# mackelab/poisson-gpfa

Hardware: AMD Instinct MI355X
Metric: EM iterations/sec (higher is better)
Workload: dtype f64

## Files before the change

poisson-gpfa_amd/csrc/core.hip:

```cpp
#include "ctx.h"
#include "model.h"
#include "dual.h"

using namespace pgpfa;

thread_local std::string g_err;
thread_local unsigned long long g_fail_count = 0;

int fail(const char* fmt, ...) {
  char buf[1024];
  va_list ap;
  va_start(ap, fmt);
  vsnprintf(buf, sizeof(buf), fmt, ap);
  va_end(ap);
  g_err = buf;
  ++g_fail_count;
  return 1;
}

int ensure_hbuf(pgpfa_ctx* c, size_t len) {
  if (len <= c->hbuf_len) return 0;
  if (c->hbuf) hipHostFree(c->hbuf);
  c->hbuf = nullptr;
  HIPC(hipHostMalloc((void**)&c->hbuf, len * sizeof(double)));
// ... 842 lines not shown
  c->info["arena_bytes"] = 0.0;
  c->info["last_eps_wt_norm"] = 0.0;
  c->info["last_eps_wt_rms"] = 0.0;
  c->info["last_split_cov"] = 0.0;
  c->info["last_syrk_tile"] = 0.0;
  c->info["last_split_sps"] = 0.0;
  c->info["last_cross_kernel"] = 0.0;
  c->info["last_mix_form"] = 0.0;
  c->info["last_yt_mix_fused"] = 0.0;
  c->info["last_cov_f32"] = 0.0;
  c->info["last_cov_f32_fallbacks"] = 0.0;
  for (const char* k : {"plan_ms_total", "plans", "set_params_calls", "last_retry_ms", "last_dense_retries", "last_param_step", "last_param_step_prev",
                        "last_fallback_no_descent", "last_fallback_line_search", "last_fallback_outer_cap", "arena_grow_ms_total", "last_cold_restarts"}) c->info[k] = 0.0;
  *out = c;
  return 0;
}

int pgpfa_destroy(pgpfa_ctx* c) {
  if (!c) return 0;
  hipSetDevice(c->device);
  if (c->st) hipStreamSynchronize(c->st);
  if (c->comm) ncclCommDestroy(c->comm);
  for (void* p : c->allocs) hipFree(p);
  if (c->vsmgp) hipFree(c->vsmgp);
  if (c->Flr32) hipFree(c->Flr32);
  if (c->lam_keep) hipFree(c->lam_keep);
  if (c->split_buf) hipFree(c->split_buf);
  if (c->Yhi) hipFree(c->Yhi);
  if (c->trial_len) hipFree(c->trial_len);
  if (c->obs) hipFree(c->obs);
  if (c->trunc_q) hipFree(c->trunc_q);
  arena_release(c);
  if (c->hbuf) hipHostFree(c->hbuf);
  if (c->dl_stage) hipHostFree(c->dl_stage);
  if (c->hibuf) hipHostFree(c->hibuf);
  if (c->ring) hipHostFree(c->ring);
  if (c->h_pcg) hipHostFree(c->h_pcg);
  if (c->h_seq) hipHostFree(c->h_seq);
  for (auto e : c->prof.pool) hipEventDestroy(e);
  if (c->st2) { hipStreamSynchronize(c->st2); hipStreamDestroy(c->st2); }
  if (c->tau_pin) hipHostFree(c->tau_pin);
  if (c->ev_tau_fork) hipEventDestroy(c->ev_tau_fork);
  if (c->ev_tau_done) hipEventDestroy(c->ev_tau_done);
  if (c->ev_fork) hipEventDestroy(c->ev_fork);
  if (c->ev_join) hipEventDestroy(c->ev_join);
  if (c->st) hipStreamDestroy(c->st);
  delete c;
  return 0;
}

int pgpfa_set_option(pgpfa_ctx* c, const char* key, double v) {
  if (!c || !key) return fail("null argument");
  const std::string k(key);
  if (k == "newton_xtol") c->xtol = v;
  else if (k == "newton_max_iter") c->max_iter = (int)v;
  else if (k == "use_mfma") {
    const bool was = c->mfma;
    c->mfma = (v != 0.0);
    if (c->have_params && c->rank_gran != 16 && was != c->mfma)
      CHK(pgpfa_set_params(c, std::vector<double>(c->hC).data(), std::vector<double>(c->hd).data(), std::vector<double>(c->htau).data()));
  }
  else if (k == "cd_mfma") c->cd_mfma = (v != 0.0);
  else if (k == "cd_hess_mfma") c->cd_hess_mfma = (v != 0.0);
  else if (k == "cross_kernel") c->cross_kernel = (v != 0.0);
  else if (k == "cd_debug") c->cd_debug = (int)v;
  else if (k == "pcg_fused") c->pcg_fused = (int)v;
  else if (k == "pcg_w32") c->pcg_w32 = (v != 0.0);
  else if (k == "pcg_form") c->pcg_form = (int)v;
  else if (k == "pcg_vec32") c->pcg_vec32 = (int)v;
  else if (k == "pcg_rx32") c->pcg_rx32 = (int)v;
  else if (k == "pcg_adapt") c->pcg_adapt = (int)v;
  else if (k == "pcg_xcd") c->pcg_xcd = (int)v;
  else if (k == "mt_fill") c->mt_fill = (int)v;
  else if (k == "overlap_factors") c->overlap_factors = (int)v;
  else if (k == "mix_slot") c->mix_slot = (int)v;
  else if (k == "yt_mix") c->yt_mix = (v != 0.0);
  else if (k == "pivchol_pairs") c->pivchol_pairs = (v != 0.0);
  else if (k == "vsm_b4") c->vsm_b4 = (int)v;
  else if (k == "poisson_tiles") c->poisson_tiles = (int)v;
  else if (k == "yt_mix_dbg") c->yt_mix_dbg = (int)v;
  else if (k == "yt_mix_dma") c->yt_mix_dma = (v != 0.0);
  else if (k == "syrk_dbg") c->syrk_dbg = (int)v;
  else if (k == "syrk_tile") c->syrk_tile = (int)v;
  else if (k == "mix_wide") c->mix_wide = (int)v;
  else if (k == "thin_products") {
    const bool was = c->thin_products >= 2;
    c->thin_products = (int)v;
    if (c->have_params && c->rank_gran != 16 && was != (c->thin_products >= 2))
      CHK(pgpfa_set_params(c, std::vector<double>(c->hC).data(), std::vector<double>(c->hd).data(), std::vector<double>(c->htau).data()));
  }
  else if (k == "copy_kernels") c->copy_kernels = (v != 0.0);
  else if (k == "chord") c->chord = (v != 0.0);
  else if (k == "shared_pcg") c->shared_pcg = (v != 0.0);
  else if (k == "time_newton") c->time_newton = (v != 0.0);
  else if (k == "pcg_trace") c->pcg_trace = (v != 0.0);
  else if (k == "measure_mix") { c->measure_mix = (v != 0.0); c->info["last_eps_wt_norm"] = 0.0; c->info["last_eps_wt_rms"] = 0.0; }
  else if (k == "pcg_retire") c->pcg_retire = (v != 0.0);
  else if (k == "split_cov") c->split_cov = (v != 0.0);
  else if (k == "split_max_norm") c->split_max_norm = v;
  else if (k == "cov_mode") c->cov_mode = (int)v;
  else if (k == "lowrank_tol") {
    const bool changed = c->lr_tol != v;
    c->lr_tol = v;
    if (c->have_params && changed)
      CHK(pgpfa_set_params(c, std::vector<double>(c->hC).data(), std::vector<double>(c->hd).data(), std::vector<double>(c->htau).data()));
  }
  else if (k == "keep_trial_vsmgp") c->keep_trial_vsmgp = (v != 0.0);
  else if (k == "dual_lowrank") c->dual_lowrank = (v != 0.0);
  else if (k == "dual_f32") c->dual_f32 = (int)v;
  else if (k == "laplace_f32") { if (v != 0.0 && v != 1.0 && v != 2.0) return fail("laplace_f32 is 0, 1 or 2"); c->laplace_f32 = (int)v; }
  else if (k == "dual_masked") { if (v != 0.0 && v != 1.0) return fail("dual_masked is 0 or 1"); c->dual_masked = (int)v; }
  else if (k == "laplace_evidence") { if (v != 0.0 && v != 1.0) return fail("laplace_evidence is 0 or 1"); c->laplace_evidence = (int)v; }
  else if (k == "sample_chunk_trials") { if (v < 0.0 || v != std::floor(v)) return fail("sample_chunk_trials is a count of trials, or 0"); c->sample_chunk = (int)v; }
  else if (k == "rates_chunk_trials") { if (v < 0.0 || v != std::floor(v)) return fail("rates_chunk_trials is a count of trials, or 0"); c->rates_chunk = (int)v; }
  else if (k == "slab_row_align") c->slab_row_align = (v != 0.0);
  else if (k == "vsm_mfma") c->vsm_mfma = (v != 0.0);
  else if (k == "dual_gemm") c->dual_gemm = (v != 0.0);
  else if (k == "extrapolate_start") c->extrapolate = (v != 0.0);
  else if (k == "extrapolate_beta") c->extrapolate_beta = v;
  else if (k == "extrapolate_guard") c->extrapolate_guard = v;
  else if (k == "start_guard") c->start_guard = (v != 0.0);
  else if (k == "shared_min") c->shared_min = (int)v;
  else if (k == "pcg_inner") c->pcg_inner_max = std::max(1, (int)v);
  else if (k == "pcg_eta0") c->pcg_eta0 = v;
  else if (k == "splitk_target") c->splitk_target = std::max(1, (int)v);
  else if (k == "small_tile_below") c->small_tile_below = (int)v;
  else if (k == "f32_tile64") c->f32_tile64 = (int)v;
  else if (k == "splitk_below64") c->splitk_below64 = (int)v;
  else if (k == "pcg_outer_max") c->pcg_outer_max = (int)v;
  else if (k == "chord_xtol") c->chord_xtol = v;
  else if (k == "chord_rho") c->chord_rho = v;
  else if (k == "chord_max_step") c->chord_max_step = v;
  else if (k == "chord_max") c->chord_max = (int)v;
  else if (k == "chunk_trials") { if (c->B > 0) return fail("chunk_trials must be set before the first E-step"); c->chunk_opt = (int)v; }
  else if (k == "workspace_headroom") c->arena_headroom = std::max(1.0, v);
  else if (k == "rank_gran") { if (v != 4.0 && v != 8.0 && v != 16.0) return fail("rank_gran is 4, 8 or 16"); c->rank_gran = (int)v; if (c->have_params) CHK(pgpfa_set_params(c, std::vector<double>(c->hC).data(), std::vector<double>(c->hd).data(), std::vector<double>(c->htau).data())); }
  else if (k == "workspace_pool") { if (c->arena_cap > 0) return fail("workspace_pool must be set before the first E-step"); c->use_pool = (v != 0.0); }
  else if (k == "workspace_grow_budget_ms") c->grow_budget_ms = v;
  else if (k == "workspace_grow_floor_slots") c->grow_floor_slots = std::max(1, (int)v);
  else if (k == "workspace_granule_mb") c->vmm_granule = (size_t)std::max(2.0, v) << 20;
  else if (k == "workspace_vmm") { if (c->arena_cap > 0) return fail("workspace_vmm must be set before the first E-step"); c->vmm = (v != 0.0) ? 0 : -1; }
  else if (k == "eps_noise") {
    const bool changed = c->eps != v;
    c->eps = v;
    if (c->have_params && changed)
      CHK(pgpfa_set_params(c, std::vector<double>(c->hC).data(), std::vector<double>(c->hd).data(), std::vector<double>(c->htau).data()));
  }
  else if (k == "profile") {
    if (v != 0.0) {
      prof_collect(c);
      c->prof.ms.clear(); c->prof.flops.clear(); c->prof.count.clear(); c->prof.max_ms.clear(); c->prof.max_flops.clear(); c->prof.shapes.clear();
      HIPC(hipSetDevice(c->device));
      const size_t want = 2 * (256 + 64) + 2;
      while (c->prof.pool.size() < want) {
        hipEvent_t e;
        HIPC(hipEventCreate(&e));
        c->prof.pool.push_back(e);
        c->prof.idle.push_back(e);
      }
      for (int rep = 0; rep < 8; ++rep)
        for (hipEvent_t e : c->prof.idle) HIPC(hipEventRecord(e, c->st));
      HIPC(hipStreamSynchronize(c->st));
    }
    c->prof.on = (v != 0.0);
    c->prof.configured = c->prof.on;
    c->prof.only_tag = (v == 2.0) ? TAG_GEMM : (v == 3.0) ? TAG_MIX : -1;
// ... 452 lines not shown
```

poisson-gpfa_amd/csrc/cov.hip:

```cpp
#include "ctx.h"
#include "model.h"
#include "split.h"
#include "ytmix.h"

using namespace pgpfa;

template <typename TIN>
void launch_post_vsm(pgpfa_ctx* c, const TIN* Mt, long long sM, int ncol, int ns, int full_range, const int* roff = nullptr, int ts = 0) {
  const int T = c->T, p = c->p;
  if (ts <= 0) ts = T;
  if (p > 10 && c->vsm_mfma) {
    const int CB = post_vsm_mfma_cb(p, sizeof(TIN) == 4);
    if (p <= 20 && c->vsm_b4) {
      constexpr int VW = 16 / (int)sizeof(TIN);
      const bool vec = c->vsm_b4 >= 2 && T % VW == 0 && ts % VW == 0 && c->ld % VW == 0 && sM % VW == 0 && (((size_t)Mt) & 15) == 0;
      auto go = [&](auto nbk, auto vv) {
        constexpr int NBK = decltype(nbk)::value;
        constexpr bool VEC = decltype(vv)::value;
        const size_t lds4 = (size_t)CB * post_vsm_b4_cs(p, VEC) * sizeof(TIN);
        constexpr int BINS = VEC ? 64 : 32;
        (void)hipFuncSetAttribute(reinterpret_cast<const void*>(&post_vsm_b4_kernel<NBK, TIN, VEC>), hipFuncAttributeMaxDynamicSharedMemorySize, (int)lds4);
        hipLaunchKernelGGL((post_vsm_b4_kernel<NBK, TIN, VEC>), dim3((T + BINS - 1) / BINS, ns), dim3(512), lds4, c->st, Mt, sM, c->ld, ncol, T, p, c->vsm,
                           c->ident, c->trial_of_slot, full_range, CB, roff, (int)GBN, ts);
      };
// ... 35 lines not shown
  }
}


int ensure_mt_clean(pgpfa_ctx* c) {
  if (!c->mt_dirty) return 0;
  HIPC(hipMemsetAsync(c->ws.Mt, 0, (size_t)c->ws.sM * c->B * sizeof(double), c->st));
  c->mt_dirty = false;
  return 0;
}

int ensure_vsmgp_buffer(pgpfa_ctx* c) {
  if (c->vsmgp) return 0;
  const size_t bytes = (size_t)c->R * c->p * c->T * c->T * sizeof(double);
  void* ptr = nullptr;
  hipError_t e = hipMalloc(&ptr, bytes);
  if (e != hipSuccess) { (void)hipGetLastError(); return fail("hipMalloc(%zu bytes) for the per-trial post_vsmGP blocks failed: %s", bytes, hipGetErrorString(e)); }
  e = hipMemsetAsync(ptr, 0, bytes, c->st);
  if (e != hipSuccess) { hipFree(ptr); return fail("hipMemset failed: %s", hipGetErrorString(e)); }
  c->vsmgp = reinterpret_cast<double*>(ptr);
  c->bytes += bytes;
  return 0;
}

int ensure_evidence_buffers(pgpfa_ctx* c) {
  if (!c->ldet_buf) CHK(dmalloc(c, &c->ldet_buf, (size_t)c->B * c->T + 16));
  if (!c->evid_ld) CHK(dmalloc(c, &c->evid_ld, (size_t)c->B));
  return 0;
}

static int posterior_blocks_dense(pgpfa_ctx* c, int nb, double diag_scale, bool want_vsmgp, double* ld_dev) {
  const int T = c->T, p = c->p;
  c->info["last_cov_f32"] = 0.0;
  CHK(ensure_mt_clean(c));
  c->last_cov_lowrank = false;
  CHK(assemble(c, c->ident, nb, diag_scale));
  CHK(factor(c, c->ws, c->ident, nb));
  if (ld_dev) {
    double ldk = 0.0;
    for (double v : c->logdetK) ldk += v;
    hipLaunchKernelGGL(evidence_logdet_kernel, dim3(nb), dim3(256), 0, c->st, (const double*)nullptr, 0, c->ws.H, (long long)c->ws.sH, c->ld, c->npad, ldk, ld_dev);
  }
  CHK(inverse_t(c, c->ws, c->ident, nb));
  if (want_vsmgp) {
    CHK(ensure_vsmgp_buffer(c));
    for (int k = 0; k < p; ++k) {
      const int kal = (k * T) / 16 * 16;
      GemmP g{};
      g.A = c->ws.Mt + (size_t)kal * c->ld + (size_t)k * T; g.sA = c->ws.sM; g.lda = c->ld;
      g.B = g.A; g.sB = c->ws.sM; g.ldb = c->ld;
      g.C = c->ws.H; g.sC = c->ws.sH; g.ldc = T;
      g.M = T; g.N = T; g.K = c->npad - kal; g.alpha = 1.0; g.beta = 0.0;
      g.slots = c->ident; g.nbatch = nb; g.mode = GEMM_LOWER; g.kflags = KF_BEGIN_MAXRC;
      CHK(gemm(c, false, g));
      hipLaunchKernelGGL(scatter_vsmgp_kernel, dim3((unsigned)(((size_t)T * T + 255) / 256), nb), dim3(256), 0, c->st, c->ws.H, c->ws.sH, c->vsmgp,
                         T, p, k, c->trial_of_slot);
    }
  }
  prof_begin(c, TAG_VSM, (double)nb * c->npad * c->npad * p);
  launch_post_vsm(c, (const double*)c->ws.Mt, (long long)c->ws.sM, c->npad, nb, 0);
  prof_end(c);
  HIPC(hipGetLastError());
  return 0;
}


constexpr int SPLIT_NS = 256;

static int split_syrk_launch(pgpfa_ctx* c, const float* D, long long sD, int ldd, int Ts, int T, int p, int ract, int nb, int sps_req, int tile_req, double* part,
                             int* tile_used, int* sps_out, int* ngroups_out) {
  const int sps = sps_req > 0 ? sps_req : std::max(1, (nb + PACC_SPLITS - 1) / PACC_SPLITS);
  const int ngroups = (nb + sps - 1) / sps;
  SyrkF16Args a{};
  a.D = D; a.sD = sD; a.ldd = ldd; a.ts = Ts; a.part = part;
  a.T = T; a.p = p; a.ract = ract; a.nslots = nb; a.sps = sps; a.ngroups = ngroups;
  a.dbg = c->syrk_dbg;
  const int t256 = (T + 255) / 256;
  const bool big = tile_req >= 256 && T > 256 && (Ts & 3) == 0 && (ldd & 3) == 0 && t256 * 256 <= Ts && (((size_t)D) & 15) == 0 && (sD & 3) == 0;
  a.tiles = big ? t256 : (T + 127) / 128; a.ntiles = a.tiles * (a.tiles + 1) / 2;
  const long long blocks = (long long)a.ntiles * ngroups * p;
  prof_begin(c, TAG_VSM, 3.0 * (double)nb * ract * T * T * p);
  if (big) {
    const size_t lds = (size_t)4 * 2 * 256 * 32 * sizeof(_Float16);
    (void)hipFuncSetAttribute(reinterpret_cast<const void*>(&syrk256_f16x2_kernel), hipFuncAttributeMaxDynamicSharedMemorySize, (int)lds);
    hipLaunchKernelGGL(syrk256_f16x2_kernel, dim3((unsigned)blocks), dim3(512), lds, c->st, a);
  } else {
    hipLaunchKernelGGL(syrk_f16x2_kernel, dim3((unsigned)blocks), dim3(256), 0, c->st, a);
  }
  prof_end(c);
  *tile_used = big ? 256 : 128;
  *sps_out = sps;
  *ngroups_out = ngroups;
  return 0;
}

static int split_latent_sums(pgpfa_ctx* c, const double* A0, long long sM, int lda, const float* Dk, long long sD, int ldd, int rk, int kw, int T, int nb, int sps,
                             bool cross, double* Spart, double* Xpart, double* Ssum, double* Xsum, int* cross_used) {
  const int ngroups = (nb + sps - 1) / sps;
  const int spsS = std::max(1, (nb + SPLIT_NS - 1) / SPLIT_NS);
  auto seg = [&](int sper, bool is_x, double* out) -> int {
    const int nfull = nb / sper, rem = nb - nfull * sper;
    for (int part = 0; part < 2; ++part) {
      const int first = part ? nfull * sper : 0, per = part ? rem : sper, ng = part ? (rem ? 1 : 0) : nfull;
      if (ng == 0 || per == 0) continue;
      GemmP g{};
      g.A = A0 + (size_t)first * sM; g.sA = (long long)per * sM; g.lda = lda;
      g.kseg = kw; g.sAseg = sM;
      g.K = per * kw; g.alpha = 1.0; g.beta = 0.0; g.slots = nullptr; g.nbatch = ng; g.kflags = 0; g.bm = 64;
      g.M = rk;
      if (is_x) {
        g.B = reinterpret_cast<const double*>(Dk + (size_t)first * sD);
        g.sB = (long long)per * sD; g.ldb = ldd; g.sBseg = sD; g.b_f32 = 1;
        g.N = T; g.mode = GEMM_FULL;
        g.C = out + (size_t)(part ? nfull : 0) * rk * T; g.sC = (long long)rk * T; g.ldc = rk;
      } else {
        g.B = g.A; g.sB = g.sA; g.ldb = lda; g.sBseg = sM;
        g.N = rk; g.mode = GEMM_LOWER;
        g.C = out + (size_t)(part ? nfull : 0) * rk * rk; g.sC = (long long)rk * rk; g.ldc = rk;
      }
      CHK(gemm(c, false, g));
    }
    return 0;
  };
  CHK(seg(spsS, false, Spart));
  const bool use_cross = cross && c->mfma && rk % 16 == 0 && kw % 16 == 0;
  if (use_cross) {
    for (int row0 = 0; row0 < rk; row0 += 128) {
      CrossArgs ca{};
      ca.A = A0; ca.sM = sM; ca.lda = lda;
      ca.D = Dk; ca.sD = sD; ca.ldd = ldd;
      ca.C = Xpart; ca.sC = (long long)rk * T;
      ca.rk = std::min(128, rk - row0); ca.T = T; ca.kw = kw; ca.nslots = nb; ca.sps = sps;
      ca.row0 = row0; ca.ldc = rk;
      prof_begin(c, TAG_GEMM, 2.0 * (double)nb * ca.rk * (double)kw * T);
      cross_term_launch<float, false>(ca, dim3((T + 63) / 64, ngroups), c->st);
      prof_end(c);
    }
    HIPC(hipGetLastError());
  } else {
    CHK(seg(sps, true, Xpart));
  }
  const int ngS = (nb + spsS - 1) / spsS;
  hipLaunchKernelGGL(sum_groups_kernel, dim3((unsigned)(((size_t)rk * rk + 63) / 64)), dim3(256), 0, c->st, Spart, ngS, rk, rk, 32, Ssum);
  hipLaunchKernelGGL(sum_groups_kernel, dim3((unsigned)(((size_t)rk * T + 63) / 64)), dim3(256), 0, c->st, Xpart, ngroups, rk, T, 0, Xsum);
  *cross_used = use_cross ? 1 : 0;
  return 0;
}

static int accumulate_split(pgpfa_ctx* c, const CholWS& lw, int nb, int ract, int Ts, bool skip_zero_cols, int ctile, bool fused) {
  const int T = c->T, p = c->p, Tp = c->Tp, rpad = c->rpad;
  const long long sW = (long long)T * p * p;
  const size_t tt = (size_t)T * T;
  (void)skip_zero_cols;
  constexpr int NS = SPLIT_NS, NG = PACC_SPLITS + 1;
  const size_t tq = (size_t)round_up(T, 16) * round_up(T, 16);
  if (!c->split_buf) {
    const size_t len = ((size_t)NS + NG + 3) * tq + 2 * (size_t)p * tt + 1024;
    if (hipMalloc((void**)&c->split_buf, len * sizeof(double)) != hipSuccess) { (void)hipGetLastError(); c->split_buf = nullptr; return fail("out of device memory for the split accumulation (%zu bytes)", len * sizeof(double)); }
    c->bytes += len * sizeof(double);
  }
  double* Spart = c->split_buf;
  double* Xpart = Spart + (size_t)NS * tq;
  double* Ssum = Xpart + (size_t)NG * tq;
  double* Xsum = Ssum + tq;
  double* Zb = Xsum + tq;
  double* T1 = Zb + tq;
  double* Xfull = T1 + (size_t)p * tt;
  float* D = reinterpret_cast<float*>(lw.H + (size_t)c->ld * rpad);
// ... 661 lines not shown
```

poisson-gpfa_amd/csrc/ctx.h:

```cpp
#pragma once
#include <hip/hip_runtime.h>
#include <rccl/rccl.h>

#include <algorithm>
#include <limits>
#include <chrono>
#include <cmath>
#include <cstdarg>
#include <cstdio>
#include <cstring>
#include <deque>
#include <functional>
#include <map>
#include <string>
#include <type_traits>
#include <vector>

#include <mutex>
#include <rocprofiler-sdk-roctx/roctx.h>
#include "../../include/pgpfa.h"
#include "types.h"

using namespace pgpfa;

// ... 118 lines not shown
  double* lam_keep = nullptr;
  int snap_serial = 0;
  double *vec = nullptr, *cdpart = nullptr, *cdout = nullptr;
  double *cdhpart = nullptr, *cdhout = nullptr, *cdcenter = nullptr, *cdpack = nullptr;
  int* last_trials = nullptr;
  std::vector<int> last_trials_h;
  bool have_counts = false, have_params = false, have_post = false, have_precomp = false;
  double n_trials_global = 0.0;
  int B = 0;
  double grow_budget_ms = 200.0;
  int grow_floor_slots = 128;
  bool use_pool = true;
  int plan_target = 0;
  int want_slots = 0;
  bool B_capped = false;
  CholWS ws{};
  double *Xc = nullptr, *Xt = nullptr, *KX = nullptr, *KD = nullptr, *Gl = nullptr, *Glt = nullptr, *Gt = nullptr, *Dl = nullptr;
  double *W = nullptr, *Wt = nullptr, *fpart = nullptr;
  double *lamd = nullptr, *dgrad = nullptr, *dpart = nullptr, *ldet_buf = nullptr;
  double* voff = nullptr;
  bool var_active = false, lam_out_active = false;
  double* dual_scr = nullptr; long long dual_sscr = 0;
  CholWS sws{};
  double *sU = nullptr, *sDinvT = nullptr, *Wbar = nullptr;
  double *Rv = nullptr, *Zv = nullptr, *Pv = nullptr, *Qv = nullptr;
  PcgCtl* pcgctl = nullptr;
  int* live = nullptr; float *pcg_ratio = nullptr, *pcg_eta = nullptr;
  int* live1 = nullptr;
  int* pcg_blk = nullptr;
  const int* cur_ndev = nullptr;
  bool live_gemm_collect = false;
  std::vector<std::pair<std::string, double>> live_gemms;
  bool pcg_retire = true;
  int* h_pcg = nullptr; int* d_hpcg = nullptr;
  float* W32 = nullptr;
  double* sc_part2 = nullptr;
  int pcg_fused = 1; bool pcg_w32 = true;
  int mt_fill = 1;
  int pcg_xcd = 1;
  int pcg_adapt = 1;
  int pcg_form = 2;
  int pcg_rx32 = 1;
  int pcg_vec32 = 1;
  double *Sv = nullptr, *cg_scal = nullptr;
  double *GbT = nullptr, *WbT = nullptr;
  double *sc_rz = nullptr, *sc_pq = nullptr, *sc_rr = nullptr, *sc_rr0 = nullptr, *sc_pack = nullptr;
  double* Flr = nullptr;
  double* Gbin = nullptr;
  int *d_rank = nullptr, *d_blk_lat = nullptr, *d_blk_col = nullptr, *d_roff = nullptr;
  int *d_kr_ft = nullptr, *d_kr_f = nullptr;
  int kr_ft_len = 0, kr_f_len = 0;
  int ntab_ft = 0, ntab_f = 0; size_t tab_cap = 0;
  int *d_thin_ft = nullptr, *d_thin_f = nullptr, *d_thin_s = nullptr;
  int nthin_ft = 0, nthin_f = 0, nthin_s = 0;
  int thin_products = 2;
  double *Fbig = nullptr, *FTbig = nullptr, *Gbar = nullptr, *Wtbar = nullptr;
  std::vector<int> rk, roff;
  std::vector<int> rr, roff16;
  int rtot = 0, rpad = 0, rtot16 = 0;
  int rank_gran = 4;
  bool rank_compact = false;
  int *d_roff16 = nullptr, *d_cmap = nullptr, *d_nrtab = nullptr;
  int cov_mode = 0;
  double lr_tol = 1e-10;
  bool plan_lowrank = false;
  size_t slab_elems = 0, mt_elems = 0, ws_mark = 0;
  char* arena = nullptr; size_t arena_cap = 0, arena_off = 0; int arena_mode = 0;
  int vmm = 0; size_t va_size = 0, vmm_gran = 0, vmm_granule = (size_t)1 << 30;
  std::vector<std::pair<hipMemGenericAllocationHandle_t, size_t>> vmm_chunks;
  double arena_headroom = 2.0;
  bool mt_dirty = false;
  bool last_cov_lowrank = false;
  bool shared_pcg = true;
  bool pcg_trace = false;
  double* zero16 = nullptr;
  double* sink = nullptr;
  int mix_wide = 1;
  int poisson_tiles = 2;
  int vsm_b4 = 2;
  int pivchol_pairs = 1;
  int yt_mix = 1;
  int syrk_tile = 256;
  int syrk_dbg = 0;
  int yt_mix_dma = 1;
  int yt_mix_dbg = 0;
  int mix_slot = 3;
  bool cross_kernel = true;
  bool measure_mix = false;
  bool time_newton = false;
  int shared_min = 16, pcg_inner_min = 2, pcg_inner_max = 16, pcg_outer_max = 12;
  double pcg_eta0 = 1e-2;
  int splitk_target = 1280;
  int f32_tile64 = 1;
  int small_tile_below = 1 << 30;
  int splitk_below64 = 400;
  double *sc_f = nullptr, *sc_qxx = nullptr, *sc_qdx = nullptr, *sc_qdd = nullptr, *sc_dec = nullptr, *sc_smax = nullptr, *sc_alpha = nullptr;
  int *trial_of_slot = nullptr, *list_a = nullptr, *list_b = nullptr, *ident = nullptr;
  int* mask_of_slot = nullptr;
  bool mask_active = false;
  CholWS kws{};
  double *tK = nullptr, *tM = nullptr, *tA1 = nullptr, *tA2 = nullptr, *tscal = nullptr, *tpart = nullptr;
  double* hbuf = nullptr; size_t hbuf_len = 0;
  struct DlEntry { void* host; size_t off, bytes; };
  PcgCtl fused_ctl_host{};
  char* dl_stage = nullptr; size_t dl_used = 0; std::vector<DlEntry> dl_pending;
  char* dl_stage_dev = nullptr; char* ring_dev = nullptr;
  unsigned* h_seq = nullptr; unsigned* d_seq = nullptr; unsigned seq_next = 0;
  bool copy_kernels = true;
  unsigned long long dl_fail_mark = 0;
  int* hibuf = nullptr; size_t hibuf_len = 0;
  char* ring = nullptr; size_t ring_slot = 0; int ring_cur = 0, ring_pending = 0;
  std::map<std::string, double> info;
  std::vector<void*> allocs;
  size_t bytes = 0;
  Prof prof;
  ncclComm_t comm = nullptr;
  int rank = 0, nranks = 1;
  double* commbuf = nullptr; size_t commbuf_len = 0;
  double* rates_tbl = nullptr; double rates_tbl_params = -1.0;
  int rates_chunk = 0;
  int sample_chunk = 0;
};

template <typename T>
int dmalloc(pgpfa_ctx* c, T** out, size_t count, bool zero = false) {
  void* p = nullptr;
  const size_t bytes = std::max<size_t>(count, 1) * sizeof(T);
  if (c->arena_mode) {
    const size_t aligned = (bytes + 255) & ~(size_t)255;
    *out = nullptr;
    if (c->arena_mode == 2) {
      if (c->arena_off + aligned > c->arena_cap) return fail("workspace arena overflow (%zu + %zu > %zu bytes)", c->arena_off, aligned, c->arena_cap);
      p = c->arena + c->arena_off;
      if (zero && hipMemsetAsync(p, 0, bytes, c->st) != hipSuccess) return fail("hipMemset failed");
      *out = reinterpret_cast<T*>(p);
    }
    c->arena_off += aligned;
    return 0;
  }
  hipError_t e = hipMalloc(&p, bytes);
  if (e != hipSuccess) return fail("hipMalloc(%zu bytes) failed: %s", bytes, hipGetErrorString(e));
  if (zero) {
    e = hipMemsetAsync(p, 0, bytes, c->st);
    if (e != hipSuccess) return fail("hipMemset failed: %s", hipGetErrorString(e));
  }
  c->allocs.push_back(p);
  c->bytes += bytes;
  *out = reinterpret_cast<T*>(p);
  return 0;
}

template <typename F>
void dispatch_pw(int p, F&& f) {
  switch (p) {
    case 1: f(std::integral_constant<int, 1>{}); break;
    case 2: f(std::integral_constant<int, 2>{}); break;
    case 3: f(std::integral_constant<int, 3>{}); break;
    case 4: f(std::integral_constant<int, 4>{}); break;
    case 5: f(std::integral_constant<int, 5>{}); break;
    case 6: f(std::integral_constant<int, 6>{}); break;
    case 7: case 8: f(std::integral_constant<int, 8>{}); break;
    case 9: case 10: f(std::integral_constant<int, 10>{}); break;
    case 11: case 12: f(std::integral_constant<int, 12>{}); break;
    case 13: case 14: case 15: case 16: f(std::integral_constant<int, 16>{}); break;
    case 17: case 18: case 19: case 20: f(std::integral_constant<int, 20>{}); break;
    default: f(std::integral_constant<int, 32>{}); break;
// ... 110 lines not shown
```

poisson-gpfa_amd/csrc/split.h:

```cpp
#pragma once
#include <type_traits>
#include <hip/hip_runtime.h>

namespace pgpfa {

typedef _Float16 half8_t __attribute__((ext_vector_type(8)));
typedef float float4v_t __attribute__((ext_vector_type(4)));

constexpr float SPLIT_SCALE = 2048.0f;


template <int PW>
__global__ __launch_bounds__(256, 2) void mix_vsm_split_kernel(const double* __restrict__ Yt, long long sY, int ldy, float* __restrict__ D, long long sD,
                                                            int ldd, const double* __restrict__ G, long long sG, int T, int p, int rpad, double eps,
                                                            double* __restrict__ vsm, const int* __restrict__ slots,
                                                            const int* __restrict__ trial_of_slot, const int* __restrict__ roff, int col_tile, int ts) {
  constexpr int PP = PW * PW, LD = PP + 1, NPAIR = PW * (PW + 1) / 2;
  __shared__ double Gs[64 * LD];
  const int pp = p * p;
  const int slot = slots[blockIdx.y];
  const int t0 = blockIdx.x * 64;
  const int nt = min(64, T - t0);
  const double* gbase = G + (size_t)slot * sG + (size_t)t0 * pp;
  if (p < PW)
// ... 449 lines not shown
    if (!stage) return;
    _Float16* Hh = is_b ? Bh[buf] : Ah[buf];
    _Float16* Hl = is_b ? Bl[buf] : Al[buf];
#pragma unroll
    for (int r = 0; r < 4; ++r) {
      half8_t h, l;
#pragma unroll
      for (int j = 0; j < 8; ++j) {
        const float x = v4[j][r] * SPLIT_SCALE;
        const _Float16 hx = (a.dbg & 1) ? (_Float16)0 : (_Float16)x;
        h[j] = hx;
        l[j] = (a.dbg & 1) ? (_Float16)0 : (_Float16)(x - (float)hx);
      }
      *reinterpret_cast<half8_t*>(&Hh[lidx(4 * rq + r, co)]) = h;
      *reinterpret_cast<half8_t*>(&Hl[lidx(4 * rq + r, co)]) = l;
    }
  };
  const int l15 = lane & 15, l4 = lane >> 4;
  auto multiply = [&](int buf) {
    if (!wave_live || (a.dbg & 2)) return;
    const _Float16* Bhs = diag ? Ah[buf] : Bh[buf];
    const _Float16* Bls = diag ? Al[buf] : Bl[buf];
    half8_t ah[4], al[4], bh[4], bl[4];
#pragma unroll
    for (int mi = 0; mi < 4; ++mi) {
      const int r = lidx(wm * 64 + mi * 16 + l15, l4);
      ah[mi] = *reinterpret_cast<const half8_t*>(&Ah[buf][r]);
      al[mi] = *reinterpret_cast<const half8_t*>(&Al[buf][r]);
    }
#pragma unroll
    for (int ni = 0; ni < 4; ++ni) {
      const int r = lidx(wn * 64 + ni * 16 + l15, l4);
      bh[ni] = *reinterpret_cast<const half8_t*>(&Bhs[r]);
      bl[ni] = *reinterpret_cast<const half8_t*>(&Bls[r]);
    }
#pragma unroll
    for (int mi = 0; mi < 4; ++mi)
#pragma unroll
      for (int ni = 0; ni < 4; ++ni) {
        acc[mi][ni] = __builtin_amdgcn_mfma_f32_16x16x32_f16(bh[ni], ah[mi], acc[mi][ni], 0, 0, 0);
        acc[mi][ni] = __builtin_amdgcn_mfma_f32_16x16x32_f16(bh[ni], al[mi], acc[mi][ni], 0, 0, 0);
        acc[mi][ni] = __builtin_amdgcn_mfma_f32_16x16x32_f16(bl[ni], ah[mi], acc[mi][ni], 0, 0, 0);
      }
  };
  auto run = [&](auto vecc) {
    if (nsteps <= 0) return;
    constexpr bool FAST = decltype(vecc)::value;
    auto ld = [&](int step, float4v_t (&v4)[8]) { if constexpr (FAST) load_fast(v4); else load(vecc, step, v4); };
    ld(0, vA);
    ld(1, vB);
    store(0, vA);
    if (!(a.dbg & 8)) __syncthreads();
    for (int step = 0; step < nsteps; step += 2) {
      ld(step + 2, vA);
      multiply(0);
      if (step + 1 < nsteps) store(1, vB);
      if (!(a.dbg & 8)) __syncthreads();
      if (step + 1 >= nsteps) break;
      ld(step + 3, vB);
      multiply(1);
      if (step + 2 < nsteps) store(0, vA);
      if (!(a.dbg & 8)) __syncthreads();
    }
  };
  if (vec) run(std::true_type{}); else run(std::false_type{});
  if (!wave_live) return;
  double* C = a.part + (size_t)(k * a.ngroups + g) * a.T * a.T;
  const double inv = 1.0 / ((double)SPLIT_SCALE * (double)SPLIT_SCALE);
#pragma unroll
  for (int mi = 0; mi < 4; ++mi) {
    const int i = i0 + wm * 64 + mi * 16 + l15;
    if (i >= a.T) continue;
#pragma unroll
    for (int ni = 0; ni < 4; ++ni)
#pragma unroll
      for (int r = 0; r < 4; ++r) {
        const int j = j0 + wn * 64 + ni * 16 + 4 * l4 + r;
        if (j >= a.T) continue;
        C[(size_t)j * a.T + i] = (double)acc[mi][ni][r] * inv;
      }
  }
}

inline __global__ __launch_bounds__(512, 1) void syrk256_f16x2_kernel(SyrkF16Args a) {
  constexpr int BT = 256, KS = 32, LS = 32;
  auto lidx = [](int row, int chunk) { return row * LS + ((chunk ^ ((4 - ((row >> 2) & 3)) & 3)) << 3); };
  extern __shared__ __attribute__((aligned(16))) _Float16 syrk256_lds[];
  _Float16* Ah = syrk256_lds;
  _Float16* Al = Ah + 2 * BT * LS;
  _Float16* Bh = Al + 2 * BT * LS;
  _Float16* Bl = Bh + 2 * BT * LS;
  const int tid = threadIdx.x;
  const int lane = tid & 63;
  const int wave = __builtin_amdgcn_readfirstlane(tid >> 6);
  const int wm = wave >> 1, wn = wave & 1;
  const int nbatch = a.ngroups * a.p;
  int b, tile;
  {
    const int bid = blockIdx.x;
    const int full = nbatch >> 3, per_group = a.ntiles << 3, grp = bid / per_group;
    if (grp < full) { const int r = bid - grp * per_group; tile = r >> 3; b = (grp << 3) + (r & 7); }
    else { const int m = nbatch - (full << 3); const int r = bid - full * per_group; tile = r / m; b = (full << 3) + (r - tile * m); }
  }
  int tj = 0, rem = tile;
  while (rem >= a.tiles - tj) { rem -= a.tiles - tj; ++tj; }
  const int ti = tj + rem;
  const int k = b / a.ngroups, g = b - k * a.ngroups;
  const int i0 = ti * BT, j0 = tj * BT;
  const bool diag = (ti == tj);
  const int s_begin = g * a.sps, s_end = min(a.nslots, s_begin + a.sps);
  const bool wave_live = (i0 + wm * 64 < a.T) && (j0 + wn * 128 < a.T) && !(i0 + wm * 64 + 63 < j0 + wn * 128);

  float4v_t acc[4][8];
#pragma unroll
  for (int mi = 0; mi < 4; ++mi)
#pragma unroll
    for (int ni = 0; ni < 8; ++ni) acc[mi][ni] = float4v_t{0.f, 0.f, 0.f, 0.f};

  const bool is_b = tid >= 256;
  const int rq = tid & 63, co = (tid >> 6) & 3;
  const int row0 = (is_b ? j0 : i0) + 4 * rq;
  const bool stage = !(is_b && diag);
  const int steps_per_slot = (a.ract + KS - 1) / KS;
  const int nsteps = (s_end - s_begin) * steps_per_slot;
  int cur_s = s_begin, cur_c = 0;
  const unsigned voff = (unsigned)(stage ? (co * 8) * a.ldd + row0 : 0) * 4u;
  float4v_t v[8];
  auto load_fast = [&]() {
    typedef unsigned u32x4 __attribute__((ext_vector_type(4)));
    const __amdgpu_buffer_rsrc_t rs = wave_uniform_rsrc(a.D + (size_t)cur_s * a.sD, (size_t)a.ract * a.ldd * sizeof(float));
    const unsigned soff = (unsigned)(k * a.ts + cur_c * KS * a.ldd) * 4u;
#pragma unroll
    for (int j = 0; j < 8; ++j) {
      const u32x4 w = __builtin_amdgcn_raw_buffer_load_b128(rs, (int)voff, (int)(soff + (unsigned)(j * a.ldd) * 4u), 0);
      v[j] = float4v_t{__uint_as_float(w.x), __uint_as_float(w.y), __uint_as_float(w.z), __uint_as_float(w.w)};
    }
    if (cur_c + 1 < steps_per_slot) ++cur_c;
    else if (cur_s + 1 < s_end) { ++cur_s; cur_c = 0; }
  };
  auto store = [&](int buf) {
    if (!stage) return;
    _Float16* Hh = (is_b ? Bh : Ah) + buf * BT * LS;
    _Float16* Hl = (is_b ? Bl : Al) + buf * BT * LS;
#pragma unroll
    for (int r = 0; r < 4; ++r) {
      half8_t h, l;
#pragma unroll
      for (int j = 0; j < 8; ++j) {
        const float x = v[j][r] * SPLIT_SCALE;
        const _Float16 hx = (_Float16)x;
        h[j] = hx;
        l[j] = (_Float16)(x - (float)hx);
      }
      *reinterpret_cast<half8_t*>(&Hh[lidx(4 * rq + r, co)]) = h;
      *reinterpret_cast<half8_t*>(&Hl[lidx(4 * rq + r, co)]) = l;
    }
  };
  const int l15 = lane & 15, l4 = lane >> 4;
  auto multiply = [&](int buf) {
    if (!wave_live) return;
    const _Float16* As_h = Ah + buf * BT * LS;
    const _Float16* As_l = Al + buf * BT * LS;
    const _Float16* Bs_h = (diag ? Ah : Bh) + buf * BT * LS;
    const _Float16* Bs_l = (diag ? Al : Bl) + buf * BT * LS;
    half8_t ah[4], al[4];
#pragma unroll
    for (int mi = 0; mi < 4; ++mi) {
      const int r = lidx(wm * 64 + mi * 16 + l15, l4);
      ah[mi] = *reinterpret_cast<const half8_t*>(&As_h[r]);
      al[mi] = *reinterpret_cast<const half8_t*>(&As_l[r]);
    }
#pragma unroll
    for (int half = 0; half < 2; ++half) {
      half8_t bh[4], bl[4];
#pragma unroll
      for (int ni = 0; ni < 4; ++ni) {
        const int r = lidx(wn * 128 + half * 64 + ni * 16 + l15, l4);
        bh[ni] = *reinterpret_cast<const half8_t*>(&Bs_h[r]);
        bl[ni] = *reinterpret_cast<const half8_t*>(&Bs_l[r]);
      }
#pragma unroll
      for (int mi = 0; mi < 4; ++mi)
#pragma unroll
        for (int ni = 0; ni < 4; ++ni) {
          float4v_t c = acc[mi][half * 4 + ni];
          c = __builtin_amdgcn_mfma_f32_16x16x32_f16(bh[ni], ah[mi], c, 0, 0, 0);
          c = __builtin_amdgcn_mfma_f32_16x16x32_f16(bh[ni], al[mi], c, 0, 0, 0);
          c = __builtin_amdgcn_mfma_f32_16x16x32_f16(bl[ni], ah[mi], c, 0, 0, 0);
          acc[mi][half * 4 + ni] = c;
        }
    }
  };
  if (nsteps > 0) {
    load_fast();
    store(0);
    __syncthreads();
    for (int step = 0; step < nsteps; ++step) {
      if (step + 1 < nsteps) load_fast();
      multiply(step & 1);
      if (step + 1 < nsteps) store((step + 1) & 1);
      __syncthreads();
    }
  }
  if (!wave_live) return;
  double* C = a.part + (size_t)(k * a.ngroups + g) * a.T * a.T;
  const double inv = 1.0 / ((double)SPLIT_SCALE * (double)SPLIT_SCALE);
#pragma unroll
  for (int mi = 0; mi < 4; ++mi) {
    const int i = i0 + wm * 64 + mi * 16 + l15;
    if (i >= a.T) continue;
#pragma unroll
    for (int ni = 0; ni < 8; ++ni)
#pragma unroll
      for (int r = 0; r < 4; ++r) {
        const int j = j0 + wn * 128 + ni * 16 + 4 * l4 + r;
        if (j >= a.T) continue;
        C[(size_t)j * a.T + i] = (double)acc[mi][ni][r] * inv;
      }
  }
}

struct CrossArgs {
  const double* A; long long sM; int lda;
  const void* D; long long sD; int ldd;
  double* C; long long sC;
  int rk, T, kw, nslots, sps;
  int row0, ldc;
};

template <int NTR, typename TB, bool LOWER>
__global__ __launch_bounds__(256) void cross_term_kernel(CrossArgs a) {
  constexpr int GK = 16;
  constexpr int RS = NTR * 16 + ((NTR & 1) ? 0 : 16);
  constexpr int NA = (GK * NTR * 16 + 255) / 256;
  __shared__ double As[2][GK][RS];
  __shared__ double Bs[2][GK][64 + 16];
  const int tid = threadIdx.x;
  const int lane = tid & 63, wave = __builtin_amdgcn_readfirstlane(tid >> 6);
  const int l15 = lane & 15, l4 = lane >> 4;
  const int t0 = blockIdx.x * 64;
  const int g = blockIdx.y;
  const int s_begin = g * a.sps, s_end = min(a.nslots, s_begin + a.sps);
  const int cps = a.kw / GK;
  const int nchunks = (s_end - s_begin) * cps;
  const int rk = a.rk;
  const TB* Dall = reinterpret_cast<const TB*>(a.D);
  const int ct = blockIdx.x * 4 + wave;
  const bool wave_live = t0 + wave * 16 < a.T;

  double raA[NA], raB[NA];
  TB rbA[4], rbB[4];
  int cur_s = s_begin, cur_c = 0;
  size_t aoff[NA], doff[4];
#pragma unroll
  for (int u = 0; u < NA; ++u) {
    const int e = tid + 256 * u;
    const int kk = min(e / (NTR * 16), GK - 1), i = min(e % (NTR * 16), rk - 1);
    aoff[u] = (size_t)kk * a.lda + i;
  }
#pragma unroll
  for (int u = 0; u < 4; ++u) {
    const int e = tid + 256 * u;
    const int kk = e >> 6, t = min(t0 + (e & 63), a.T - 1) - t0;
    doff[u] = (size_t)kk * a.ldd + t;
  }
  auto load = [&](int, double (&ra)[NA], TB (&rb)[4]) {
    const int c0 = cur_c * GK;
    const double* Ap = a.A + (size_t)cur_s * a.sM + (size_t)c0 * a.lda + a.row0;
    const TB* Dp = Dall + (size_t)cur_s * a.sD + (size_t)c0 * a.ldd + t0;
#pragma unroll
    for (int u = 0; u < NA; ++u) ra[u] = Ap[aoff[u]];
#pragma unroll
    for (int u = 0; u < 4; ++u) rb[u] = Dp[doff[u]];
    if (cur_c + 1 < cps) ++cur_c;
    else if (cur_s + 1 < s_end) { ++cur_s; cur_c = 0; }
  };
  auto store = [&](int buf, const double (&ra)[NA], const TB (&rb)[4]) {
#pragma unroll
    for (int u = 0; u < NA; ++u) {
      const int e = tid + 256 * u;
      const int kk = e / (NTR * 16), i = e - kk * (NTR * 16);
      if (kk < GK) As[buf][kk][i] = (i < rk) ? ra[u] : 0.0;
    }
#pragma unroll
// ... 148 lines not shown
```

Baseline: 12.45.

## Software-pipeline the 256-tile f16x2 SYRK kernel, interleaving loads, splits and MFMAs

After: 12.47 (median of 3 runs). No clear change (+0.1%).

```diff
diff --git a/poisson-gpfa_amd/csrc/core.hip b/poisson-gpfa_amd/csrc/core.hip
--- a/poisson-gpfa_amd/csrc/core.hip
+++ b/poisson-gpfa_amd/csrc/core.hip
@@ -948,6 +948,7 @@
   else if (k == "yt_mix_dma") c->yt_mix_dma = (v != 0.0);
   else if (k == "syrk_dbg") c->syrk_dbg = (int)v;
   else if (k == "syrk_tile") c->syrk_tile = (int)v;
+  else if (k == "syrk_pipe") c->syrk_pipe = (v != 0.0);
   else if (k == "mix_wide") c->mix_wide = (int)v;
   else if (k == "thin_products") {
     const bool was = c->thin_products >= 2;
diff --git a/poisson-gpfa_amd/csrc/cov.hip b/poisson-gpfa_amd/csrc/cov.hip
--- a/poisson-gpfa_amd/csrc/cov.hip
+++ b/poisson-gpfa_amd/csrc/cov.hip
@@ -141,8 +141,10 @@
   prof_begin(c, TAG_VSM, 3.0 * (double)nb * ract * T * T * p);
   if (big) {
     const size_t lds = (size_t)4 * 2 * 256 * 32 * sizeof(_Float16);
-    (void)hipFuncSetAttribute(reinterpret_cast<const void*>(&syrk256_f16x2_kernel), hipFuncAttributeMaxDynamicSharedMemorySize, (int)lds);
-    hipLaunchKernelGGL(syrk256_f16x2_kernel, dim3((unsigned)blocks), dim3(512), lds, c->st, a);
+    void (*kern)(SyrkF16Args) = c->syrk_pipe ? (a.dbg ? &syrk256_f16x2_kernel<true, true> : &syrk256_f16x2_kernel<true, false>)
+                                             : (a.dbg ? &syrk256_f16x2_kernel<false, true> : &syrk256_f16x2_kernel<false, false>);
+    (void)hipFuncSetAttribute(reinterpret_cast<const void*>(kern), hipFuncAttributeMaxDynamicSharedMemorySize, (int)lds);
+    hipLaunchKernelGGL(kern, dim3((unsigned)blocks), dim3(512), lds, c->st, a);
   } else {
     hipLaunchKernelGGL(syrk_f16x2_kernel, dim3((unsigned)blocks), dim3(256), 0, c->st, a);
   }
diff --git a/poisson-gpfa_amd/csrc/ctx.h b/poisson-gpfa_amd/csrc/ctx.h
--- a/poisson-gpfa_amd/csrc/ctx.h
+++ b/poisson-gpfa_amd/csrc/ctx.h
@@ -224,6 +224,7 @@
   int yt_mix = 1;
   int syrk_tile = 256;
   int syrk_dbg = 0;
+  int syrk_pipe = 1;
   int yt_mix_dma = 1;
   int yt_mix_dbg = 0;
   int mix_slot = 3;
diff --git a/poisson-gpfa_amd/csrc/split.h b/poisson-gpfa_amd/csrc/split.h
--- a/poisson-gpfa_amd/csrc/split.h
+++ b/poisson-gpfa_amd/csrc/split.h
@@ -555,8 +555,11 @@
   }
 }
 
-inline __global__ __launch_bounds__(512, 1) void syrk256_f16x2_kernel(SyrkF16Args a) {
+template <bool PIPE, bool DBG>
+__global__ __launch_bounds__(512, 1) void syrk256_f16x2_kernel(SyrkF16Args a) {
   constexpr int BT = 256, KS = 32, LS = 32;
+  const bool no_cvt = DBG && (a.dbg & 1), no_mul = DBG && (a.dbg & 2), no_bar = DBG && (a.dbg & 8);
+  auto sync = [&]() { if (!no_bar) __syncthreads(); };
   auto lidx = [](int row, int chunk) { return row * LS + ((chunk ^ ((4 - ((row >> 2) & 3)) & 3)) << 3); };
   extern __shared__ __attribute__((aligned(16))) _Float16 syrk256_lds[];
   _Float16* Ah = syrk256_lds;
@@ -599,17 +602,24 @@
   int cur_s = s_begin, cur_c = 0;
   const unsigned voff = (unsigned)(stage ? (co * 8) * a.ldd + row0 : 0) * 4u;
   float4v_t v[8];
-  auto load_fast = [&]() {
+  auto load_cols = [&](auto j0c, auto nc) __attribute__((always_inline)) {
     typedef unsigned u32x4 __attribute__((ext_vector_type(4)));
+    constexpr int J0 = decltype(j0c)::value, N = decltype(nc)::value;
     const __amdgpu_buffer_rsrc_t rs = wave_uniform_rsrc(a.D + (size_t)cur_s * a.sD, (size_t)a.ract * a.ldd * sizeof(float));
     const unsigned soff = (unsigned)(k * a.ts + cur_c * KS * a.ldd) * 4u;
 #pragma unroll
-    for (int j = 0; j < 8; ++j) {
+    for (int j = J0; j < J0 + N; ++j) {
       const u32x4 w = __builtin_amdgcn_raw_buffer_load_b128(rs, (int)voff, (int)(soff + (unsigned)(j * a.ldd) * 4u), 0);
       v[j] = float4v_t{__uint_as_float(w.x), __uint_as_float(w.y), __uint_as_float(w.z), __uint_as_float(w.w)};
     }
+  };
+  auto advance = [&]() __attribute__((always_inline)) {
     if (cur_c + 1 < steps_per_slot) ++cur_c;
     else if (cur_s + 1 < s_end) { ++cur_s; cur_c = 0; }
+  };
+  auto load_fast = [&]() {
+    load_cols(std::integral_constant<int, 0>{}, std::integral_constant<int, 8>{});
+    advance();
   };
   auto store = [&](int buf) {
     if (!stage) return;
@@ -621,17 +631,100 @@
 #pragma unroll
       for (int j = 0; j < 8; ++j) {
         const float x = v[j][r] * SPLIT_SCALE;
-        const _Float16 hx = (_Float16)x;
+        const _Float16 hx = no_cvt ? (_Float16)0 : (_Float16)x;
         h[j] = hx;
-        l[j] = (_Float16)(x - (float)hx);
+        l[j] = no_cvt ? (_Float16)0 : (_Float16)(x - (float)hx);
       }
       *reinterpret_cast<half8_t*>(&Hh[lidx(4 * rq + r, co)]) = h;
       *reinterpret_cast<half8_t*>(&Hl[lidx(4 * rq + r, co)]) = l;
     }
   };
   const int l15 = lane & 15, l4 = lane >> 4;
+  constexpr unsigned STAGE_BYTES = BT * LS * sizeof(_Float16);
+  char* lds_bytes = reinterpret_cast<char*>(syrk256_lds);
+  unsigned a_off = (unsigned)lidx(wm * 64 + l15, l4) * 2u;
+  unsigned b_off = (diag ? 0u : 4u * STAGE_BYTES) + (unsigned)lidx(wn * 128 + l15, l4) * 2u;
+  unsigned w_off = (is_b ? 4u * STAGE_BYTES : 0u) + STAGE_BYTES + (unsigned)lidx(4 * rq, co) * 2u;
+  auto pipe_step = [&](auto livec, auto n1c, auto n2c) __attribute__((always_inline)) {
+    constexpr bool LIVE = decltype(livec)::value, N1 = decltype(n1c)::value, N2 = decltype(n2c)::value;
+    typedef _Float16 half4_t __attribute__((ext_vector_type(4)));
+    const _Float16* As_h = reinterpret_cast<const _Float16*>(lds_bytes + a_off);
+    const _Float16* As_l = As_h + 2 * BT * LS;
+    const _Float16* Bs_h = reinterpret_cast<const _Float16*>(lds_bytes + b_off);
+    const _Float16* Bs_l = Bs_h + 2 * BT * LS;
+    _Float16* Hh = reinterpret_cast<_Float16*>(lds_bytes + w_off);
+    _Float16* Hl = Hh + 2 * BT * LS;
+    half8_t ah[4], al[4], bh, bl;
+    half4_t ph[4], pl[4];
+    auto split1 = [&](float d, _Float16& h, _Float16& l) __attribute__((always_inline)) {
+      const float x = d * SPLIT_SCALE;
+      const _Float16 hx = no_cvt ? (_Float16)0 : (_Float16)x;
+      h = hx;
+      l = no_cvt ? (_Float16)0 : (_Float16)(x - (float)hx);
+    };
+    if constexpr (LIVE) {
+      bh = *reinterpret_cast<const half8_t*>(&Bs_h[0]);
+#pragma unroll
+      for (int mi = 0; mi < 4; ++mi) {
+        ah[mi] = *reinterpret_cast<const half8_t*>(&As_h[mi * 16 * LS]);
+        al[mi] = *reinterpret_cast<const half8_t*>(&As_l[mi * 16 * LS]);
+      }
+    }
+#pragma unroll
+    for (int c = 0; c < 8; ++c) {
+      if constexpr (LIVE) {
+        bl = *reinterpret_cast<const half8_t*>(&Bs_l[c * 16 * LS]);
+#pragma unroll
+        for (int mi = 0; mi < 4; ++mi) acc[mi][c] = __builtin_amdgcn_mfma_f32_16x16x32_f16(bh, ah[mi], acc[mi][c], 0, 0, 0);
+#pragma unroll
+        for (int mi = 0; mi < 4; ++mi) acc[mi][c] = __builtin_amdgcn_mfma_f32_16x16x32_f16(bh, al[mi], acc[mi][c], 0, 0, 0);
+      }
+      if constexpr (N1) {
+        if (c == 0 || c == 2) {
+#pragma unroll
+          for (int j = c; j < c + 2; ++j)
+#pragma unroll
+            for (int r = 0; r < 4; ++r) {
+              _Float16 h, l;
+              split1(v[j][r], h, l);
+              ph[r][j] = h;
+              pl[r][j] = l;
+            }
+        } else if (c == 4 || c == 5) {
+#pragma unroll
+          for (int r = 2 * (c - 4); r < 2 * (c - 4) + 2; ++r) {
+            half8_t h, l;
+#pragma unroll
+            for (int j = 0; j < 4; ++j) { h[j] = ph[r][j]; l[j] = pl[r][j]; }
+#pragma unroll
+            for (int j = 4; j < 8; ++j) {
+              _Float16 hh, ll;
+              split1(v[j][r], hh, ll);
+              h[j] = hh;
+              l[j] = ll;
+            }
+            *reinterpret_cast<half8_t*>(&Hh[r * LS]) = h;
+            *reinterpret_cast<half8_t*>(&Hl[r * LS]) = l;
+          }
+        }
+      }
+      if constexpr (N2) {
+        if (c == 0) load_cols(std::integral_constant<int, 0>{}, std::integral_constant<int, 2>{});
+        if (c == 2) load_cols(std::integral_constant<int, 2>{}, std::integral_constant<int, 2>{});
+        if (c == 5) { load_cols(std::integral_constant<int, 4>{}, std::integral_constant<int, 4>{}); advance(); }
+      }
+      __builtin_amdgcn_sched_barrier(0);
+      if constexpr (LIVE) {
+        if (c + 1 < 8) bh = *reinterpret_cast<const half8_t*>(&Bs_h[(c + 1) * 16 * LS]);
+#pragma unroll
+        for (int mi = 0; mi < 4; ++mi) acc[mi][c] = __builtin_amdgcn_mfma_f32_16x16x32_f16(bl, ah[mi], acc[mi][c], 0, 0, 0);
+        __builtin_amdgcn_sched_barrier(0);
+      }
+    }
+    a_off ^= STAGE_BYTES; b_off ^= STAGE_BYTES; w_off ^= STAGE_BYTES;
+  };
   auto multiply = [&](int buf) {
-    if (!wave_live) return;
+    if (!wave_live || no_mul) return;
     const _Float16* As_h = Ah + buf * BT * LS;
     const _Float16* As_l = Al + buf * BT * LS;
     const _Float16* Bs_h = (diag ? Ah : Bh) + buf * BT * LS;
@@ -664,15 +757,39 @@
         }
     }
   };
-  if (nsteps > 0) {
+  if constexpr (PIPE) {
+    if (nsteps > 0) {
+      constexpr std::true_type yes{};
+      constexpr std::false_type no{};
+      const bool live = wave_live && !no_mul;
+      const bool stage_w = !(wave >= 4 && diag);
+      auto run = [&](auto livec, auto stagec) __attribute__((always_inline)) {
+        int step = 0;
+        if constexpr (decltype(stagec)::value) {
+          for (; step + 2 < nsteps; ++step) { pipe_step(livec, yes, yes); sync(); }
+          if (step + 1 < nsteps) { pipe_step(livec, yes, no); sync(); }
+        } else {
+          for (; step + 1 < nsteps; ++step) { pipe_step(livec, no, no); sync(); }
+        }
+        pipe_step(livec, no, no);
+        sync();
+      };
+      load_fast();
+      store(0);
+      if (nsteps > 1) load_fast();
+      sync();
+      if (live) { if (stage_w) run(yes, yes); else run(yes, no); }
+      else { if (stage_w) run(no, yes); else run(no, no); }
+    }
+  } else if (nsteps > 0) {
     load_fast();
     store(0);
-    __syncthreads();
+    sync();
     for (int step = 0; step < nsteps; ++step) {
       if (step + 1 < nsteps) load_fast();
       multiply(step & 1);
       if (step + 1 < nsteps) store((step + 1) & 1);
-      __syncthreads();
+      sync();
     }
   }
   if (!wave_live) return;
```
